# JihyongOh/DeMFI

Measured on AMD Instinct MI355X. Metric: interpolated frames/sec @720p x8 MFI (N_tst=3), higher is better.
Workload: dtype f16; 1 GPU; DeMFI-Net_rb N_tst=3, x8 MFI, 720x1280 (padded 736x1280), fp16, clip-parallel windows, random-init weights; uint8 frames host->HBM->host inside the timed region (PNG codec excluded), 8 distinct windows; graph=True, parallelism=clip1, n_ctx=7, n_trunk=3

## Files before the change

### demfi_amd/_lib.py

```python
import ctypes as C
import os

_HERE = os.path.dirname(os.path.abspath(__file__))
LIB_PATH = os.environ.get('DEMFI_HIP_LIB') or os.path.join(_HERE, 'csrc', 'libdemfi_hip.so')

F16, F32 = 0, 1
ABI_VERSION = 8
ACT_NONE, ACT_RELU, ACT_TANH, ACT_SIGMOID = 0, 1, 2, 3
MODE_STORE, MODE_MUL, MODE_GRU = 0, 1, 2
BT601, BT709 = 0, 1
SITING_420JPEG, SITING_420MPEG2 = 0, 1
YUV_LAYOUT = {'420': 0, '422': 1, '444': 2, 'mono': 3}
MAX_PIECES, MAX_CHUNKS, MAX_SEGS, MAX_OCTS = 48, 40, 8, 32


class View(C.Structure):
    _fields_ = [('ptr', C.c_void_p), ('sx', C.c_int64), ('sy', C.c_int64), ('sc', C.c_int64), ('sb', C.c_int64),
                ('is_f32', C.c_int32), ('_pad', C.c_int32)]


class Piece(C.Structure):
    _fields_ = [('v', View), ('nch', C.c_int32), ('lds_ch', C.c_int32), ('up_shift', C.c_int32), ('fat', C.c_int32)]


class Chunk(C.Structure):
    _fields_ = [('first_piece', C.c_int32), ('n_pieces', C.c_int32), ('nks', C.c_int32), ('_pad', C.c_int32),
                ('w_off', C.c_int64)]


class Seg(C.Structure):
    _fields_ = [('dst', View), ('res', View), ('aux', View), ('act', C.c_int32), ('mode', C.c_int32),
                ('scale', C.c_int32), ('dy', C.c_int32), ('dx', C.c_int32), ('_pad', C.c_int32)]


class Conv(C.Structure):
    _fields_ = [('dtype', C.c_int32), ('H', C.c_int32), ('W', C.c_int32), ('inH', C.c_int32), ('inW', C.c_int32),
                ('kh', C.c_int32), ('kw', C.c_int32), ('stride', C.c_int32), ('pad_y', C.c_int32),
                ('pad_x', C.c_int32), ('batch', C.c_int32), ('cout_pad', C.c_int32), ('nco', C.c_int32),
                ('rec_bytes', C.c_int32), ('n_chunks', C.c_int32), ('n_pieces', C.c_int32), ('n_segs', C.c_int32),
                ('cout_perm', C.c_int32), ('w_blk_stride', C.c_int64), ('wpack', C.c_void_p), ('bias', C.c_void_p), ('zero_page', C.c_void_p),
                ('chunks', Chunk * MAX_CHUNKS), ('pieces', Piece * MAX_PIECES), ('segs', Seg * MAX_SEGS),
                ('oct_seg', C.c_int32 * MAX_OCTS), ('oct_n', C.c_int32 * MAX_OCTS), ('oct_ch', C.c_int32 * MAX_OCTS),
                ('sub_seg', C.c_int32 * (MAX_OCTS // 4)),
                ('lw_magic', C.c_uint32), ('u8_iter', C.c_int32), ('u8_sink', C.c_void_p),
                ('pack', View), ('pack_oct_ch', C.c_int32 * 4)]


class U8Sink(C.Structure):
    _fields_ = [('frame', C.c_void_p * MAX_SEGS), ('h', C.c_int32), ('w', C.c_int32), ('iter', C.c_int32), ('_pad', C.c_int32)]


class ConvSrc(C.Structure):
    _fields_ = [('v', View), ('fat', C.c_int32), ('up_shift', C.c_int32), ('nch', C.c_int32), ('_pad', C.c_int32),
                ('cin', C.POINTER(C.c_int32))]


class ConvDst(C.Structure):
    _fields_ = [('dst', View), ('res', View), ('aux', View), ('act', C.c_int32), ('mode', C.c_int32), ('scale', C.c_int32),
                ('dy', C.c_int32), ('dx', C.c_int32), ('n', C.c_int32), ('couts', C.POINTER(C.c_int32))]


class HParams(C.Structure):
    _fields_ = [('nf', C.c_int32), ('scale_factor', C.c_int32), ('num_resb_facfb', C.c_int32), ('num_resb_dec', C.c_int32),
                ('shared_fgac', C.c_int32), ('fgac_rr', C.c_int32), ('fgac_sr', C.c_int32), ('flags', C.c_int32)]


class Batch(C.Structure):
    _fields_ = [('nb', C.c_int32), ('_pad', C.c_int32), ('a', C.c_int64), ('b', C.c_int64), ('o', C.c_int64), ('t', C.c_int64),
                ('p', C.c_int64 * 32)]


class Op(C.Structure):
    _fields_ = [('kind', C.c_int32), ('conv', C.c_int32), ('nch', C.c_int32), ('_pad', C.c_int32), ('macs', C.c_int64),
                ('a', View), ('b', View), ('o', View), ('p', C.c_void_p * 32), ('t', C.c_void_p), ('name', C.c_char * 64),
                ('bt', Batch)]


_SIGS = {
    'demfi_abi_version': (C.c_int, []),
    'demfi_last_error': (C.c_char_p, []),
    'demfi_device_info': (C.c_int, [C.c_char_p, C.c_int, C.POINTER(C.c_int), C.POINTER(C.c_int64)]),
    'demfi_pack_conv_weights': (C.c_int, [C.c_void_p, C.c_int, C.c_int, C.c_int, C.c_int, C.c_void_p, C.c_int,
                                          C.c_void_p, C.c_int, C.c_void_p, C.c_int, C.c_int, C.c_int, C.c_void_p,
                                          C.POINTER(C.c_int64)]),
    'demfi_conv_lds_bytes': (C.c_int64, [C.POINTER(Conv)]),
# ... 166 lines not shown
```

### demfi_amd/csrc/common.h

```cpp
#pragma once
#include <hip/hip_runtime.h>
#include <stdint.h>
#include <stdio.h>
#include "demfi_hip.h"

typedef _Float16 half_t;
typedef _Float16 h8_t __attribute__((ext_vector_type(8)));
typedef _Float16 h4_t __attribute__((ext_vector_type(4)));
typedef float f16x_t __attribute__((ext_vector_type(16)));
typedef float f4_t __attribute__((ext_vector_type(4)));

int demfi_set_error(int code, const char* fmt, ...);

struct demfi_conv;
bool demfi_persist_eligible(const demfi_conv* h);
bool demfi_ws2_eligible(const demfi_conv* h);
int demfi_ws2_launch(const demfi_conv* h, const demfi_conv* dev, void* stream);
#define DEMFI_HIP_CHECK(expr)                                                                   \
    do {                                                                                        \
        hipError_t e__ = (expr);                                                                \
        if (e__ != hipSuccess)                                                                  \
            return demfi_set_error(DEMFI_ERR_HIP, "%s failed: %s", #expr, hipGetErrorString(e__)); \
    } while (0)

#define DEMFI_GLOBAL __attribute__((address_space(1)))
template <typename T> __device__ __forceinline__ const DEMFI_GLOBAL T* gcp(const void* p) { return (const DEMFI_GLOBAL T*)p; }
template <typename T> __device__ __forceinline__ DEMFI_GLOBAL T* gp(void* p) { return (DEMFI_GLOBAL T*)p; }
typedef unsigned int u4_t __attribute__((ext_vector_type(4)));
__device__ __forceinline__ uint4 ld_global16(const void* p) { return __builtin_bit_cast(uint4, *gcp<u4_t>(p)); }
__device__ __forceinline__ void st_global16(void* p, const uint4& v) { *gp<u4_t>(p) = __builtin_bit_cast(u4_t, v); }
__device__ __forceinline__ void st_global16_nt(void* p, const uint4& v) { __builtin_nontemporal_store(__builtin_bit_cast(u4_t, v), gp<u4_t>(p)); }

__device__ __forceinline__ float view_load(const demfi_view& v, int64_t off)
{
    return v.is_f32 ? gcp<float>(v.ptr)[off] : (float)gcp<half_t>(v.ptr)[off];
}
__device__ __forceinline__ void view_store(const demfi_view& v, int64_t off, float x)
{
    if (v.is_f32) gp<float>(v.ptr)[off] = x;
    else gp<half_t>(v.ptr)[off] = (half_t)x;
}

__device__ __forceinline__ float sigmoidf_(float x) { return 1.0f / (1.0f + expf(-x)); }

__device__ __forceinline__ float fast_sigmoid(float x)
{
    return __builtin_amdgcn_rcpf(1.0f + __builtin_amdgcn_exp2f(-1.4426950408889634f * x));
}
__device__ __forceinline__ float fast_tanh(float x)
{
    return 1.0f - 2.0f * __builtin_amdgcn_rcpf(1.0f + __builtin_amdgcn_exp2f(2.8853900817779268f * x));
}

__device__ __forceinline__ float unnormalized_coord(float p, float den, float sizem1)
{
    float g = (2.0f * p) / den;
    g = g - 1.0f;
    float i = (g + 1.0f) / 2.0f;
    return i * sizem1;
}

struct SampleMap {
    int x0, y0;
    float w[4];
    int inb;
};

__device__ __forceinline__ SampleMap make_sample_map(float ix, float iy, int H, int W)
{
    SampleMap m;
// ... 30 lines not shown
```

### demfi_amd/csrc/conv.hip

```cpp
#include "conv_common.h"

namespace {

bool sep_eligible(const demfi_conv* h) { return demfi_sep_eligible(h); }
bool wstream_eligible(const demfi_conv* h, int ks = 7, int nch = 2) { return demfi_wstream_eligible(h, ks, nch); }

static bool persist_out_eligible(const demfi_conv* h, bool allow_tanh = false);

bool persist_eligible(const demfi_conv* h)
{
    if (h->dtype != DEMFI_F16 || h->stride != 1 || h->kh != 3 || h->kw != 3 || h->pad_y != 1 || h->pad_x != 1) return false;
    if (h->n_chunks != 1 || h->n_pieces != 1 || h->chunks[0].nks != 4 || h->rec_bytes != 128) return false;
    const demfi_piece& p = h->pieces[0];
    if (!p.fat || p.nch != 64 || p.up_shift != 0 || !p.v.ptr || p.v.is_f32) return false;
    return persist_out_eligible(h, h->nco == 2);
}

static bool thin_out_eligible(const demfi_conv* h)
{
    if (h->nco != 1 || h->cout_pad != 32 || !h->zero_page || h->inH != h->H || h->inW != h->W || h->sub_seg[0] >= 0) return false;
    bool any = false;
    for (int g = 0; g < 4; ++g) {
        if (h->oct_n[g] == 0) continue;
        any = true;
        const demfi_seg& sg = h->segs[h->oct_seg[g]];
        if (sg.mode != DEMFI_MODE_STORE || sg.scale != 1 || sg.dy != 0 || sg.dx != 0) return false;
        if (!sg.dst.ptr || !sg.dst.is_f32) return false;
        if (sg.res.ptr && !sg.res.is_f32) return false;
    }
    return any;
}

static bool narrow_eligible(const demfi_conv* h)
{
    if (h->dtype != DEMFI_F16 || h->stride != 1 || h->kh != h->kw || (h->kh != 3 && h->kh != 7) || h->pad_y != h->kh / 2 || h->pad_x != h->kw / 2)
        return false;
    if (h->n_chunks != 1) return false;
    const demfi_chunk& ch = h->chunks[0];
    if (ch.nks != 1 && ch.nks != 2 && ch.nks != 4) return false;
    if (h->kh == 7 && (ch.nks != 1 || h->nco != 1)) return false;
    int nreal = 0;
    for (int k = 0; k < ch.n_pieces; ++k) {
        const demfi_piece& p = h->pieces[ch.first_piece + k];
        if ((p.lds_ch * 2) % 16 || (p.nch * 2) % 16) return false;
        if (p.v.ptr == nullptr) continue;
        if (!p.fat || p.up_shift != 0 || p.v.is_f32 || p.v.sc != 1) return false;
        if (p.v.sy * 2 * 16 >= (int64_t)1 << 31 || p.v.sx * 2 * 64 >= (int64_t)1 << 31) return false;
        ++nreal;
    }
    if (nreal < 1 || nreal > 2) return false;
    return persist_out_eligible(h) || thin_out_eligible(h);
}

static bool persist_out_eligible(const demfi_conv* h, bool allow_tanh)
{
    if (h->nco > 2 || h->cout_pad != 32 * h->nco || !h->zero_page || h->inH != h->H || h->inW != h->W) return false;
    const int sg = h->sub_seg[0];
    if (sg < 0) return false;
    for (int sb = 0; sb < h->nco; ++sb)
        if (h->sub_seg[sb] != sg || h->oct_ch[sb * 4] != h->oct_ch[0] + 32 * sb) return false;
    const demfi_seg& seg = h->segs[sg];
    if (seg.mode != DEMFI_MODE_STORE || seg.scale != 1 || seg.dy != 0 || seg.dx != 0) return false;
    if (seg.act != DEMFI_ACT_NONE && seg.act != DEMFI_ACT_RELU && !(allow_tanh && seg.act == DEMFI_ACT_TANH)) return false;
    return true;
}

}


bool demfi_persist_eligible(const demfi_conv* h)
{
    return sep_eligible(h) || wstream_eligible(h) || wstream_eligible(h, 3, 1) || persist_eligible(h) || (narrow_eligible(h) && persist_out_eligible(h)) ||
           demfi_ws2_eligible(h);
}

extern "C" int64_t demfi_conv_lds_bytes(const demfi_conv* h)
{
    const int64_t LW = (int64_t)(TW - 1) * h->stride + h->kw;
    const int64_t LH = (int64_t)(TH - 1) * h->stride + h->kh;
    const int64_t tile = ((LW * LH * (h->rec_bytes + REC_PAD) + 1023) & ~1023ll)
                         + 2ll * (h->rec_bytes / 32) * h->nco * 1024;
    const int64_t stage = 4 * 64 * STAGE_LD * 4;
    return tile > stage ? tile : stage;
}

extern "C" int demfi_conv2d(const demfi_conv* h, const demfi_conv* dev, void* stream)
{
    if (!h || !dev) return demfi_set_error(DEMFI_ERR_ARG, "demfi_conv2d: null descriptor");
    if (h->dtype != DEMFI_F16 && h->dtype != DEMFI_F32) return demfi_set_error(DEMFI_ERR_ARG, "demfi_conv2d: dtype");
    if (h->stride != 1 && h->stride != 2) return demfi_set_error(DEMFI_ERR_ARG, "demfi_conv2d: stride %d", h->stride);
    if (h->cout_pad <= 0 || h->cout_pad > 256 || h->cout_pad % (32 * h->nco))
        return demfi_set_error(DEMFI_ERR_ARG, "demfi_conv2d: cout_pad=%d nco=%d", h->cout_pad, h->nco);
    if (h->rec_bytes != 32 && h->rec_bytes != 64 && h->rec_bytes != 128)
        return demfi_set_error(DEMFI_ERR_ARG, "demfi_conv2d: rec_bytes=%d", h->rec_bytes);
    if (h->n_chunks < 1 || h->n_chunks > DEMFI_MAX_CHUNKS || h->n_pieces > DEMFI_MAX_PIECES || h->n_segs > DEMFI_MAX_SEGS)
        return demfi_set_error(DEMFI_ERR_ARG, "demfi_conv2d: chunk/piece/seg count");
    const int64_t LW = (int64_t)(TW - 1) * h->stride + h->kw;
    const int64_t lds = demfi_conv_lds_bytes(h);
    if (lds > 160 * 1024) return demfi_set_error(DEMFI_ERR_ARG, "demfi_conv2d: LDS tile %lld B > 160 KiB", (long long)lds);
    if (LW * ((int64_t)(TH - 1) * h->stride + h->kh) >= 65536) return demfi_set_error(DEMFI_ERR_ARG, "demfi_conv2d: tile too large");
    if (h->lw_magic != (uint32_t)((0x100000000ull + LW - 1) / LW))
        return demfi_set_error(DEMFI_ERR_ARG, "demfi_conv2d: lw_magic mismatch");
    const int esz = h->dtype == DEMFI_F16 ? 2 : 4;
    for (int c = 0; c < h->n_chunks; ++c) {
        const demfi_chunk& ch = h->chunks[c];
        if (ch.nks < 1 || ch.nks * 32 > h->rec_bytes) return demfi_set_error(DEMFI_ERR_ARG, "demfi_conv2d: chunk %d nks", c);
        int used = 0;
        for (int pi = ch.first_piece; pi < ch.first_piece + ch.n_pieces; ++pi) {
            const demfi_piece& p = h->pieces[pi];
            if (p.lds_ch * esz != used) return demfi_set_error(DEMFI_ERR_ARG, "demfi_conv2d: piece %d not contiguous in chunk", pi);
            if (p.fat) {
                const int bytes = p.nch * esz, vpp = bytes / 16;
                if (bytes % 16 || (vpp & (vpp - 1)) || vpp > 8 || p.v.sc != 1 || (p.v.is_f32 != (h->dtype == DEMFI_F32)))
                    return demfi_set_error(DEMFI_ERR_ARG, "demfi_conv2d: fat piece %d malformed", pi);
            }
            used += p.nch * esz;
        }
        if (used != ch.nks * 32) return demfi_set_error(DEMFI_ERR_ARG, "demfi_conv2d: chunk %d covers %d B, expected %d", c, used, ch.nks * 32);
    }
    for (int sb = 0; sb < h->cout_pad / 32; ++sb) {
        const int sgi = h->sub_seg[sb];
        if (sgi < 0) continue;
        if (sgi >= h->n_segs) return demfi_set_error(DEMFI_ERR_ARG, "demfi_conv2d: sub_seg[%d]=%d", sb, sgi);
        const demfi_seg& sg = h->segs[sgi];
        const int f32 = h->dtype == DEMFI_F32;
        bool ok = sg.dst.ptr && sg.dst.sc == 1 && sg.dst.is_f32 == f32;
        if (sg.res.ptr) ok = ok && sg.res.sc == 1 && sg.res.is_f32 == f32;
        if (sg.mode == DEMFI_MODE_GRU) ok = ok && sg.aux.ptr && sg.aux.sc == 1 && sg.aux.is_f32 == f32;
        if (sg.mode != DEMFI_MODE_STORE) ok = ok && sg.res.ptr;
        for (int o = 0; o < 4; ++o)
            ok = ok && h->oct_seg[sb * 4 + o] == sgi && h->oct_n[sb * 4 + o] == 8 &&
                 h->oct_ch[sb * 4 + o] == h->oct_ch[sb * 4] + 8 * o;
        ok = ok && h->oct_ch[sb * 4] % 8 == 0;
        if (!ok) return demfi_set_error(DEMFI_ERR_ARG, "demfi_conv2d: subtile %d is not eligible for the staged epilogue", sb);
    }
    hipStream_t st = (hipStream_t)stream;
    if (h->pack.ptr != nullptr) {
        bool ok = h->dtype == DEMFI_F16 && narrow_eligible(h) && thin_out_eligible(h) && !persist_out_eligible(h) && h->pack.sc == 1 && !h->pack.is_f32;
        for (int g = 0; g < 4; ++g) ok = ok && (h->pack_oct_ch[g] < 0 || (h->pack_oct_ch[g] % 4 == 0 && h->oct_n[g] > 0));
        if (!ok) return demfi_set_error(DEMFI_ERR_ARG, "demfi_conv2d: packed copy (demfi_conv.pack) on a layer that is not a thin-output fp16 narrow layer, or malformed");
    }
    if ((h->cout_perm != 0) != demfi_persist_eligible(h))
        return demfi_set_error(DEMFI_ERR_ARG, h->cout_perm ? "demfi_conv2d: descriptor packed for a persistent kernel (cout_perm) but not eligible for one (zero_page missing?)"
                                                           : "demfi_conv2d: persistent-kernel layer without cout_perm (build the descriptor with demfi_conv_build)");
    if (sep_eligible(h)) return demfi_sep_launch(h, dev, st);
    if (wstream_eligible(h)) return demfi_wstream_launch(h, dev, st);
    if (!persist_eligible(h) && !narrow_eligible(h) && demfi_ws2_eligible(h)) return demfi_ws2_launch(h, dev, st);
    if (wstream_eligible(h, 3, 1)) return demfi_wstream3_launch(h, dev, st);
    if (persist_eligible(h)) return demfi_c64_launch(h, dev, st);
    if (narrow_eligible(h)) {
        bool handled = false;
        const int rc = demfi_narrow_launch(h, dev, st, !persist_out_eligible(h), &handled);
        if (handled) return rc;
    }
    return demfi_conv_general_launch(h, dev, st, (size_t)lds);
}

#ifdef DEMFI_TRACE
extern "C" int demfi_trace_dump(unsigned long long* out, int64_t n)
{
    const int64_t have = (int64_t)TR_WGS * TR_WAVES * TR_TILES * TR_STAMPS;
    if (!out || n < have) return demfi_set_error(DEMFI_ERR_ARG, "demfi_trace_dump: need room for %lld entries", (long long)have);
    DEMFI_HIP_CHECK(hipDeviceSynchronize());
    for (int64_t i = 0; i < have; ++i) out[i] = 0;
    int st = demfi_c64_trace_collect(out);
    if (st >= 0) st = demfi_narrow_trace_collect(out);
    if (st >= 0) st = demfi_sep_trace_collect(out);
    if (st >= 0) st = demfi_wstream_trace_collect(out);
    return st < 0 ? st : (int)have;
}
#endif
```

### demfi_amd/csrc/ctx.cpp

```cpp
#include "common.h"
#include <algorithm>
#include <map>
#include <set>
#include <string>
#include <stdlib.h>
#include <string.h>
#include <vector>

namespace {

constexpr int64_t LDS_BUDGET = 78 * 1024;

struct BuiltConv {
    demfi_conv d;
    std::vector<uint8_t> wpack;
    std::vector<float> bias;
    int64_t wbytes = 0;
    int64_t macs = 0;
};

int build_conv(int dtype, int H, int W, int stride, int batch, const float* w, const float* bias, int cout, int cin, int kh,
               int kw, const demfi_conv_src* srcs, int n_srcs, const demfi_conv_dst* dsts, int n_dsts, BuiltConv& out,
               bool size_only, const char* name, int pad_y = -1, int pad_x = -1, int grid_div = 1)
{
    if (dtype != DEMFI_F16 && dtype != DEMFI_F32) return demfi_set_error(DEMFI_ERR_ARG, "%s: dtype", name);
    if (!srcs || !dsts || n_srcs <= 0 || n_dsts <= 0 || n_dsts > DEMFI_MAX_SEGS || (stride != 1 && stride != 2))
        return demfi_set_error(DEMFI_ERR_ARG, "%s: sources / destinations / stride", name);
    const int esz = dtype == DEMFI_F32 ? 4 : 2;
    const int64_t LH = 7 * stride + kh, LW = 31 * stride + kw;
    int n_oct = 0;
    for (int i = 0; i < n_dsts; ++i) n_oct += (dsts[i].n + 7) / 8;
    const int sub = (n_oct + 3) / 4;
    int nco = sub <= 5 ? sub : 4;
    int rec = 128;
    int src_nch = 0;
    for (int i = 0; i < n_srcs; ++i) src_nch += srcs[i].nch;
    const bool ws2_s2 = stride == 2 && kh == 4 && kw == 4, ws2_s1 = stride == 1 && kh == 3 && kw == 3 && src_nch > 64;
    bool ws2_shape = esz == 2 && (ws2_s2 || ws2_s1) && pad_y < 0 && pad_x < 0 && n_dsts == 1 && dsts[0].n % 64 == 0 &&
                     dsts[0].mode == DEMFI_MODE_STORE && (dsts[0].act == DEMFI_ACT_NONE || dsts[0].act == DEMFI_ACT_RELU) && dsts[0].scale <= 1 &&
                     dsts[0].dst.sc == 1 && !dsts[0].dst.is_f32 && (!dsts[0].res.ptr || (dsts[0].res.sc == 1 && !dsts[0].res.is_f32));
    for (int i = 0; ws2_shape && i < n_srcs; ++i)
        ws2_shape = srcs[i].fat && !srcs[i].v.is_f32 &&
                    (srcs[i].nch % 32 == 0 || (srcs[i].nch == 16 && !srcs[i].up_shift && (i == n_srcs - 1 || (i == n_srcs - 2 && srcs[n_srcs - 1].nch == 8))) ||
                     (srcs[i].nch == 8 && !srcs[i].up_shift && i == n_srcs - 1 && i > 0 && srcs[i - 1].nch == 16)) &&
                    (srcs[i].up_shift == 0 || (srcs[i].up_shift == 1 && ws2_s1 && H % 2 == 0 && W % 2 == 0));
    if (ws2_shape) nco = 2;
    bool sep = esz == 2 && stride == 1 && ((kh == 1 && kw == 5) || (kh == 5 && kw == 1)) && n_srcs == 2 && (cout == 64 || cout == 128);
    for (int i = 0; sep && i < n_srcs; ++i) sep = srcs[i].fat && srcs[i].nch == 64 && !srcs[i].up_shift;
    while (!sep && rec > 32 && LH * LW * (rec + 16) + 2 * (rec / 32) * nco * 1024 > LDS_BUDGET) rec /= 2;
    {
        const int64_t n_wg = (int64_t)((W + 31) / 32) * ((H + 7) / 8) * (batch / grid_div) * ((sub + nco - 1) / nco);
        const bool persist_shape = n_srcs == 1 && srcs[0].fat && srcs[0].nch == 64 && kh == 3 && kw == 3 && stride == 1;
        if (!sep && !persist_shape && rec == 128 && nco <= 2 && n_wg <= 5 * 256) rec = 64;
        bool rdb_shape = !sep && esz == 2 && kh == 3 && kw == 3 && stride == 1 && sub == 1 && n_dsts == 1 && dsts[0].n == 32 && cin >= 96 && pad_y < 0 && pad_x < 0;
        for (int i = 0; rdb_shape && i < n_srcs; ++i) rdb_shape = srcs[i].fat && !srcs[i].up_shift && srcs[i].nch % 32 == 0;
        if (rdb_shape || ws2_shape) rec = 64;
    }

    {
        std::vector<int> seen(cin, 0);
        for (int i = 0; i < n_srcs; ++i)
            for (int j = 0; j < srcs[i].nch; ++j) {
                const int c = srcs[i].cin[j];
                if (c >= cin) return demfi_set_error(DEMFI_ERR_ARG, "%s: input map names channel %d >= cin %d", name, c, cin);
                if (c >= 0) seen[c]++;
            }
        for (int c = 0; c < cin; ++c)
            if (seen[c] != 1) return demfi_set_error(DEMFI_ERR_ARG, "%s: input channel %d fed %d times", name, c, seen[c]);
    }
    struct P { demfi_view v; int nch, lds_ch, up, fat; };
    struct Ck { int first, n, nks; };
    std::vector<P> pieces;
    std::vector<Ck> chunks;
    std::vector<int32_t> cin_map;
    int first = 0, fill = 0;
    const demfi_view null_view = {nullptr, 0, 0, 0, 0, 0, 0};
    auto close_chunk = [&]() {
        if (fill == 0) return;
        const int unit = ws2_shape ? 64 : 32;
        const int padb = (unit - fill % unit) % unit;
        if (padb) {
            pieces.push_back({null_view, padb / esz, fill / esz, 0, 0});
            cin_map.insert(cin_map.end(), padb / esz, -1);
            fill += padb;
        }
        chunks.push_back({first, (int)pieces.size() - first, fill / 32});
        first = (int)pieces.size();
        fill = 0;
    };
    std::vector<int> order;
    for (int i = 0; i < n_srcs; ++i) if (srcs[i].fat) order.push_back(i);
    for (int i = 0; i < n_srcs; ++i) if (!srcs[i].fat) order.push_back(i);
    for (int si : order) {
        const demfi_conv_src& s = srcs[si];
        const int selt = s.v.is_f32 ? 4 : 2;
        int done = 0;
        while (done < s.nch) {
            if (fill >= rec) close_chunk();
            const int room = (rec - fill) / esz;
// ... 975 lines not shown
        OpList& th = tb > 1 ? c->tb_head_ops[k] : c->head_ops[k][q];
        const int H = c->H, W = c->W, N = c->N;
        const int H2 = H / 2, W2 = W / 2, H4 = H / 4, W4 = W / 4, H8 = H / 8, W8 = W / 8;
        const int R = DEMFI_ACT_RELU, T = DEMFI_ACT_TANH;
        const int64_t hw4 = (int64_t)H * W * 4;
        const Tensor& ffo = TB["ffo"];
        const Tensor& aF = TB["aF"];
        const Tensor& x = TB["x"];
        const void* tp = ptr(B["t"]);
        auto delta_v = [&](int step, int ch) { return tview(B["delta"], 5 * step + ch); };
        auto delta_p = [&](int step, int ch) { return plane(B["delta"], 5 * step + ch); };
        {
            demfi_op o = blank();
            o.p[0] = ptr(ffo); o.p[1] = ptr(ffo) + 2 * hw4; o.p[2] = ptr(B["cfr_acc"]); o.p[3] = ptr(B["ft"]); o.t = tp;
            o.p[4] = ptr(ffo) + 4 * hw4; o.p[5] = ptr(B["misc16"]);
            simple(th, DEMFI_OP_CFR, "cfr", o);
        }
        warp(th, "warp_fat", 64, fview(TB["F01"], 0, 0), fview(TB["F01"], 0, 1), fview(B["Ft"], 0, 0), ptr(B["ft"]), ptr(B["ft"]) + 2 * hw4,
             ptr(ffo) + 4 * hw4, nullptr, tp);
        std::string p = "Refine_Module.";
        {
            std::vector<int32_t> m = range(192, 201);
            m.insert(m.end(), 7, -1);
            if (c->dtype == DEMFI_F16) {
                std::vector<int32_t> sel = range(128, 201), m2 = range(64, 73);
                m2.insert(m2.end(), 7, -1);
                SubW wb = sub_weight(p + "enc1", sel, false);
                conv(th, p + "enc1#t", {fsrc(B["Ft"], 0), fsrc_map(B["misc16"], m2)},
                     {D(fview(B["u1"]), range(0, 64), R, DEMFI_MODE_STORE, fview(TB["u1a"]))}, H2, W2, 2, 1, &wb.w, &wb.b, &wb.shape);
            } else
            conv(th, p + "enc1", {fsrc(aF, 0, 0, -1, 0), fsrc(aF, 64, 0, -1, 1), fsrc(B["Ft"], 128), fsrc_map(B["misc16"], m)},
                 {D(fview(B["u1"]), range(0, 64), R)}, H2, W2, 2);
        }
        conv(th, p + "enc2", {fsrc(B["u1"], 0)}, {D(fview(B["u2"]), range(0, 128), R)}, H4, W4, 2);
        conv(th, p + "enc3", {fsrc(B["u2"], 0)}, {D(fview(B["u3"]), range(0, 256), R)}, H8, W8, 2);
        conv(th, p + "dec0", {fsrc(B["u3"], 0)}, {D(fview(B["d0"]), range(0, 256), R)}, H8, W8);
        conv(th, p + "dec1", {fsrc(B["d0"], 0, 0, -1, -1, 1), fsrc(B["u2"], 256)}, {D(fview(B["d1"]), range(0, 128), R)}, H4, W4);
        conv(th, p + "dec2", {fsrc(B["d1"], 0, 0, -1, -1, 1), fsrc(B["u1"], 128)}, {D(fview(B["d2"]), range(0, 64), R)}, H2, W2);
        if (c->dtype == DEMFI_F16) {
            auto it = c->table.find(p + "dec3");
            const Layer l3 = it->second;
            auto iw = c->weights.find(p + "dec3.weight"), ib = c->weights.find(p + "dec3.bias");
            if (!dry && (iw == c->weights.end() || ib == c->weights.end())) {
                status = demfi_set_error(DEMFI_ERR_ARG, "demfi_ctx_bind: weight '%s' was not loaded", (p + "dec3").c_str());
                return;
            }
            auto phase_view = [&](demfi_view v, int dy, int dx) {
                const int64_t elt = v.is_f32 ? 4 : 2;
                v.ptr = (char*)v.ptr + ((int64_t)dy * v.sy + (int64_t)dx * v.sx) * elt;
                v.sx *= 2; v.sy *= 2;
                return v;
            };
            const Layer l9 = {l3.cout, l3.cin, 3, 3};
            for (int dy = 0; dy < 2 && status >= 0; ++dy) {
                std::vector<float> wf2, bf2;
                for (int dx = 0; dx < 2 && status >= 0; ++dx) {
                    std::vector<float> w9e, b2;
                    if (!dry) {
                        w9e.assign((size_t)l3.cout * l3.cin * 9, 0.0f);
                        for (int co = 0; co < l3.cout; ++co)
                            for (int ci = 0; ci < l3.cin; ++ci) {
                                const float* w9 = &iw->second.data[((size_t)co * l3.cin + ci) * 9];
                                float* we = &w9e[((size_t)co * l3.cin + ci) * 9];
                                for (int ky = 0; ky < 3; ++ky)
                                    for (int kx = 0; kx < 3; ++kx) {
                                        const int a = dy == 0 ? (ky >= 1) : (ky >= 2), b = dx == 0 ? (kx >= 1) : (kx >= 2);
                                        we[(a + dy) * 3 + (b + dx)] += w9[ky * 3 + kx];
                                    }
                            }
                        b2 = ib->second.data;
                    }
                    const std::string nm = p + "dec3#p" + std::to_string(dy) + std::to_string(dx);
                    auto slice = [&](int c0, int c1, std::vector<float>& w, std::vector<float>& b) {
                        if (dry) return;
                        w.assign(w9e.begin() + (size_t)c0 * l3.cin * 9, w9e.begin() + (size_t)c1 * l3.cin * 9);
                        b.assign(b2.begin() + c0, b2.begin() + c1);
                    };
                    std::vector<float> wa, ba, wb, bb, wf, bf;
                    slice(5, 69, wa, ba); slice(69, 133, wb, bb); slice(0, 5, wf, bf);
                    const Layer l64 = {64, l3.cin, 3, 3};
                    conv(th, nm + "a", {fsrc(B["d2"], 0)},
                         {D(phase_view(fview(B["rF"], 0, 0), dy, dx), range(0, 64), T, DEMFI_MODE_STORE, phase_view(fview(aF, 0, 0), dy, dx))},
                         H2, W2, 1, 1, &wa, &ba, &l64);
                    conv(th, nm + "b", {fsrc(B["d2"], 0)},
                         {D(phase_view(fview(B["rF"], 0, 1), dy, dx), range(0, 64), T, DEMFI_MODE_STORE, phase_view(fview(aF, 0, 1), dy, dx))},
                         H2, W2, 1, 1, &wb, &bb, &l64);
                    wf2.insert(wf2.end(), wf.begin(), wf.end());
                    bf2.insert(bf2.end(), bf.begin(), bf.end());
                }
                if (status >= 0) {
                    const Layer l10 = {10, l3.cin, 3, 3};
                    pack_next(phase_view(fview(B["delta16"]), dy, 0), 0, 4, 16, 20);
                    conv(th, p + "dec3#p" + std::to_string(dy) + "xf", {fsrc(B["d2"], 0)},
                         {D(phase_view(delta_v(0, 0), dy, 0), range(0, 4), DEMFI_ACT_NONE, DEMFI_MODE_STORE, phase_view(tview(B["ft"]), dy, 0)),
                          D(phase_view(delta_v(0, 4), dy, 0), {4}, DEMFI_ACT_NONE, DEMFI_MODE_STORE, phase_view(tview(ffo, 4), dy, 0)),
                          D(phase_view(delta_v(0, 0), dy, 1), range(5, 9), DEMFI_ACT_NONE, DEMFI_MODE_STORE, phase_view(tview(B["ft"]), dy, 1)),
                          D(phase_view(delta_v(0, 4), dy, 1), {9}, DEMFI_ACT_NONE, DEMFI_MODE_STORE, phase_view(tview(ffo, 4), dy, 1))},
                         H2, W2, 1, 1, &wf2, &bf2, &l10);
                }
            }
        } else
        conv(th, p + "dec3", {fsrc(B["d2"], 0, 0, -1, -1, 1)},
             {D(fview(B["rF"], 0, 0), range(5, 69), T, DEMFI_MODE_STORE, fview(aF, 0, 0)),
              D(fview(B["rF"], 0, 1), range(69, 133), T, DEMFI_MODE_STORE, fview(aF, 0, 1)),
              D(delta_v(0, 0), range(0, 4), DEMFI_ACT_NONE, DEMFI_MODE_STORE, tview(B["ft"])),
              D(delta_v(0, 4), {4}, DEMFI_ACT_NONE, DEMFI_MODE_STORE, tview(ffo, 4))}, H, W);
        warp(th, "warp_fat", 64, fview(B["rF"], 0, 0), fview(B["rF"], 0, 1), fview(B["rF"], 0, 2), delta_p(0, 0), delta_p(0, 2),
             delta_p(0, 4), plane(B["occ"], 0), tp);
        conv(th, "Dec_first", {fsrc(B["rF"], 0)}, {D(fview(B["dec_a"]), range(0, 64), R)}, H, W, 1, 3);
        const Tensor* cur = resblocks(th, "Decoder_res", c->hp.num_resb_dec, B["dec_a"], B["dec_t"], B["dec_b"], H, W, 3);
        conv(th, "Dec_last1", {fsrc(*cur, 0)}, {D(fview(B["dec_t"]), range(0, 64), R)}, H, W, 1, 3);
        conv(th, "Dec_last2", {fsrc(B["dec_t"], 0)}, {D(tview(B["sharp1"], 0, 3ll * H * W), range(0, 3))}, H, W, 1, 3);
        conv(th, "Ch_Reducer", {fsrc(B["rF"], 0, 0, -1, 0), fsrc(B["rF"], 64, 0, -1, 1), fsrc(B["rF"], 128, 0, -1, 2)},
             {D(fview(B["frec0"]), range(0, 64), T)}, H, W);
        p = "Booster_Module.";
        std::vector<const float*> xpl;
        for (int f = 0; f < 4; ++f)
            for (int col = 0; col < 3; ++col) xpl.push_back(plane(x, col * 4 + f));
        std::vector<int32_t> agg3s_cin = range(0, 6);
        if (c->dtype == DEMFI_F16) {
            std::vector<const float*> pl;
            for (int i = 0; i < 9; ++i) pl.push_back(plane(B["sharp1"], i));
            for (int i = 0; i < 5; ++i) pl.push_back(delta_p(0, i));
            pl.push_back(plane(B["occ"], 0));
            pack(th, pl, B["ref16"]);
            std::vector<int32_t> sel = range(0, 9), m = range(0, 14);
            for (int i = 25; i < 30; ++i) sel.push_back(i);
            m.insert(m.end(), 2, -1);
            SubW w1 = sub_weight(p + "Mixer.conv_ref1", sel, true);
            conv(th, p + "Mixer.conv_ref1#t", {fsrc_map(B["ref16"], m)}, {D(fview(B["re1"]), range(0, 32), R, DEMFI_MODE_STORE, fview(TB["re1w"]))},
                 H, W, 1, 1, &w1.w, &w1.b, &w1.shape);
        } else {
            {
                std::vector<const float*> pl;
                for (int i = 0; i < 9; ++i) pl.push_back(plane(B["sharp1"], i));
                pl.insert(pl.end(), xpl.begin(), xpl.end());
                for (int i : {2, 3, 0, 1}) pl.push_back(plane(ffo, i));
                for (int i = 0; i < 5; ++i) pl.push_back(delta_p(0, i));
                pack(th, pl, B["ref32"]);
                std::vector<int32_t> m = range(0, 30);
                m.insert(m.end(), 2, -1);
// ... 713 lines not shown
```

### demfi_amd/csrc/wsconv.hip

```cpp
#include "common.h"
#include <type_traits>
#include <stdlib.h>
#include <string.h>

namespace {

template <int I, int N, typename F>
__device__ __forceinline__ void ws_for(F&& f)
{
    if constexpr (I < N) {
        f(std::integral_constant<int, I>{});
        ws_for<I + 1, N>(f);
    }
}
__device__ __forceinline__ void ws_mma(f16x_t& acc, const uint4& a, const uint4& b)
{
    acc = __builtin_amdgcn_mfma_f32_32x32x16_f16(__builtin_bit_cast(h8_t, a), __builtin_bit_cast(h8_t, b), acc, 0, 0, 0);
}

template <bool S2, int NCH = 2> struct Ws2Cfg {
    static constexpr int KSE = S2 ? 2 : 3;
    static constexpr int RPW = 8;
    static constexpr int TH = RPW * (4 / NCH), TWP = 32;
    static constexpr int LH = TH + KSE - 1, LL = TWP + KSE - 1;
// ... 444 lines not shown
        k.res = sg.res.ptr ? (const char*)sg.res.ptr + (int64_t)ch0 * 2 : nullptr;
        k.r_sb = sg.res.sb * 2; k.r_sx = (int)(sg.res.sx * 2); k.r_sy = (int)(sg.res.sy * 2);
        k.relu = sg.act == DEMFI_ACT_RELU;
    }
    for (int c = 0; c < h->n_chunks; ++c) {
        const demfi_chunk& ch = h->chunks[c];
        const demfi_piece& p = h->pieces[ch.first_piece];
        WsChunk& k = a.ch[c];
        k.src = (const char*)p.v.ptr; k.sb = p.v.sb * 2; k.sx = (int)(p.v.sx * 2); k.sy = (int)(p.v.sy * 2);
        k.flags = (p.nch == 16 ? 1 : 0) | (p.up_shift ? 2 : 0);
        k.w_off = (int)(ch.w_off * 16);
        if (ch.n_pieces == 3) {
            const demfi_piece& q = h->pieces[ch.first_piece + 1];
            k.src2 = (const char*)q.v.ptr; k.sb2 = q.v.sb * 2; k.sx2 = (int)(q.v.sx * 2); k.sy2 = (int)(q.v.sy * 2);
        }
    }
    const int grid = total >= 256 ? 256 : (int)total;
    static const bool tracing = getenv("DEMFI_WS2_TRACE") && atoi(getenv("DEMFI_WS2_TRACE")) != 0;
    static unsigned long long* trbuf = nullptr;
    if (tracing) {
        if (!trbuf) { DEMFI_HIP_CHECK(hipMalloc(&trbuf, 8 * 512 * 8)); }
        DEMFI_HIP_CHECK(hipMemset(trbuf, 0, 8 * 512 * 8));
        a.trace = trbuf;
    }
    constexpr int lds_s2 = Ws2Cfg<true, 2>::LDS_BYTES, lds_3 = Ws2Cfg<false, 2>::LDS_BYTES, lds_31 = Ws2Cfg<false, 1>::LDS_BYTES;
    if (h->stride == 2) {
        DEMFI_LDS_ATTR((conv_ws2_kernel<true, 2>));
        hipLaunchKernelGGL((conv_ws2_kernel<true, 2>), dim3(grid), dim3(WS_NTHREADS), lds_s2, (hipStream_t)stream, a);
    } else if (nco == 2) {
        DEMFI_LDS_ATTR((conv_ws2_kernel<false, 2>));
        hipLaunchKernelGGL((conv_ws2_kernel<false, 2>), dim3(grid), dim3(WS_NTHREADS), lds_3, (hipStream_t)stream, a);
    } else {
        DEMFI_LDS_ATTR((conv_ws2_kernel<false, 1>));
        hipLaunchKernelGGL((conv_ws2_kernel<false, 1>), dim3(grid), dim3(WS_NTHREADS), lds_31, (hipStream_t)stream, a);
    }
    DEMFI_HIP_CHECK(hipGetLastError());
    if (tracing) {
        static unsigned long long host[8 * 512];
        DEMFI_HIP_CHECK(hipStreamSynchronize((hipStream_t)stream));
        DEMFI_HIP_CHECK(hipMemcpy(host, trbuf, sizeof(host), hipMemcpyDeviceToHost));
        for (int w : {0, 4}) {
            fprintf(stderr, "[ws2 trace] stride %d chunks %d blocks %d wave %d:", h->stride, h->n_chunks, h->cout_pad / (32 * nco), w);
            unsigned long long prev = 0;
            for (int i = 0; i < 512 && host[w * 512 + i]; ++i) {
                const unsigned long long t = host[w * 512 + i] & 0xffffffffffffffull;
                fprintf(stderr, " %d:%lld", (int)(host[w * 512 + i] >> 56), prev ? (long long)(t - prev) : 0ll);
                prev = t;
            }
            fprintf(stderr, "\n");
        }
    }
    return DEMFI_OK;
}
```

### include/demfi_hip.h

```cpp
#ifndef DEMFI_HIP_H
#define DEMFI_HIP_H

#include <stdint.h>

#ifdef __cplusplus
extern "C" {
#endif

#define DEMFI_ABI_VERSION 8

enum demfi_dtype { DEMFI_F16 = 0, DEMFI_F32 = 1 };

enum demfi_status {
    DEMFI_OK = 0,
    DEMFI_ERR_ARG = -1,
    DEMFI_ERR_HIP = -2,
    DEMFI_ERR_NODEV = -3
};

enum demfi_yuv_matrix { DEMFI_BT601 = 0, DEMFI_BT709 = 1 };
enum demfi_chroma_siting { DEMFI_420JPEG = 0, DEMFI_420MPEG2 = 1 };
enum demfi_yuv_layout { DEMFI_YUV_420 = 0, DEMFI_YUV_422 = 1, DEMFI_YUV_444 = 2, DEMFI_YUV_MONO = 3 };

enum demfi_act { DEMFI_ACT_NONE = 0, DEMFI_ACT_RELU = 1, DEMFI_ACT_TANH = 2, DEMFI_ACT_SIGMOID = 3 };

enum demfi_mode { DEMFI_MODE_STORE = 0, DEMFI_MODE_MUL = 1, DEMFI_MODE_GRU = 2 };

typedef struct demfi_view {
    void*   ptr;
    int64_t sx;
    int64_t sy;
    int64_t sc;
    int64_t sb;
    int32_t is_f32;
    int32_t _pad;
} demfi_view;

typedef struct demfi_piece {
    demfi_view v;
    int32_t nch;
    int32_t lds_ch;
    int32_t up_shift;
    int32_t fat;
} demfi_piece;

#define DEMFI_MAX_PIECES 48
#define DEMFI_MAX_CHUNKS 40
#define DEMFI_MAX_SEGS    8
#define DEMFI_MAX_OCTS   32

typedef struct demfi_chunk {
    int32_t first_piece;
    int32_t n_pieces;
    int32_t nks;
    int32_t _pad;
    int64_t w_off;
} demfi_chunk;

typedef struct demfi_seg {
    demfi_view dst;
    demfi_view res;
    demfi_view aux;
    int32_t act;
    int32_t mode;
    int32_t scale;
    int32_t dy, dx;
    int32_t _pad;
} demfi_seg;

typedef struct demfi_conv {
    int32_t dtype;
    int32_t H, W;
    int32_t inH, inW;
    int32_t kh, kw;
    int32_t stride;
    int32_t pad_y, pad_x;
    int32_t batch;
    int32_t cout_pad;
    int32_t nco;
    int32_t rec_bytes;
    int32_t n_chunks;
    int32_t n_pieces;
    int32_t n_segs;
    int32_t cout_perm;
    int64_t w_blk_stride;
    const void*  wpack;
    const float* bias;
    const void*  zero_page;
    demfi_chunk chunks[DEMFI_MAX_CHUNKS];
    demfi_piece pieces[DEMFI_MAX_PIECES];
    demfi_seg   segs[DEMFI_MAX_SEGS];
    int32_t oct_seg[DEMFI_MAX_OCTS];
    int32_t oct_n[DEMFI_MAX_OCTS];
    int32_t oct_ch[DEMFI_MAX_OCTS];
    int32_t sub_seg[DEMFI_MAX_OCTS / 4];
    uint32_t lw_magic;
    int32_t  u8_iter;
    const struct demfi_u8_sink* u8_sink;
    demfi_view pack;
    int32_t pack_oct_ch[4];
} demfi_conv;

#define DEMFI_U8_SINK_STRIDE 256
typedef struct demfi_u8_sink {
    uint8_t* frame[DEMFI_MAX_SEGS];
    int32_t  h, w;
    int32_t  iter;
    int32_t  _pad;
} demfi_u8_sink;

int         demfi_abi_version(void);
const char* demfi_last_error(void);
int         demfi_device_info(char* name, int len, int* n_cu, int64_t* hbm_bytes);

int demfi_pack_conv_weights(const float* w_oihw, int cout, int cin, int kh, int kw,
                            const int32_t* cin_map, int n_k, const int32_t* chunk_nks, int n_chunks,
                            const int32_t* cout_map, int cout_pad, int nco, int dtype,
                            void* out, int64_t* out_bytes);

int64_t demfi_conv_lds_bytes(const demfi_conv* host_desc);
// ... 224 lines not shown
```

Before: 104.1 frames/s.

## Fuse dec3 phase convs into one 256-channel kernel sharing the input tile

For each output row parity, the two per-column-phase 64-channel dec3 convolutions (a and b) for both column phases are merged into a single 256-output conv. A new MFMA kernel stages the input tile into LDS once, then loops over four 64-channel blocks, each using its own 2x2 tap footprint, fused residual add and tanh. The goal is to cut repeated input loads and kernel launches across the four separate convs. It adds a new segment field and a dedicated, narrowly eligible kernel path, and the old path stays available through an environment variable.

```diff
diff --git a/demfi_amd/_lib.py b/demfi_amd/_lib.py
--- a/demfi_amd/_lib.py
+++ b/demfi_amd/_lib.py
@@ -30,7 +30,7 @@
 
 class Seg(C.Structure):
     _fields_ = [('dst', View), ('res', View), ('aux', View), ('act', C.c_int32), ('mode', C.c_int32),
-                ('scale', C.c_int32), ('dy', C.c_int32), ('dx', C.c_int32), ('_pad', C.c_int32)]
+                ('scale', C.c_int32), ('dy', C.c_int32), ('dx', C.c_int32), ('taps2x2', C.c_int32)]
 
 
 class Conv(C.Structure):
diff --git a/demfi_amd/csrc/common.h b/demfi_amd/csrc/common.h
--- a/demfi_amd/csrc/common.h
+++ b/demfi_amd/csrc/common.h
@@ -16,6 +16,8 @@
 bool demfi_persist_eligible(const demfi_conv* h);
 bool demfi_ws2_eligible(const demfi_conv* h);
 int demfi_ws2_launch(const demfi_conv* h, const demfi_conv* dev, void* stream);
+bool demfi_dec3_eligible(const demfi_conv* h);
+int demfi_dec3_launch(const demfi_conv* h, const demfi_conv* dev, void* stream);
 #define DEMFI_HIP_CHECK(expr)                                                                   \
     do {                                                                                        \
         hipError_t e__ = (expr);                                                                \
diff --git a/demfi_amd/csrc/conv.hip b/demfi_amd/csrc/conv.hip
--- a/demfi_amd/csrc/conv.hip
+++ b/demfi_amd/csrc/conv.hip
@@ -71,7 +71,7 @@
 bool demfi_persist_eligible(const demfi_conv* h)
 {
     return sep_eligible(h) || wstream_eligible(h) || wstream_eligible(h, 3, 1) || persist_eligible(h) || (narrow_eligible(h) && persist_out_eligible(h)) ||
-           demfi_ws2_eligible(h);
+           demfi_ws2_eligible(h) || demfi_dec3_eligible(h);
 }
 
 extern "C" int64_t demfi_conv_lds_bytes(const demfi_conv* h)
@@ -146,6 +146,7 @@
     if (sep_eligible(h)) return demfi_sep_launch(h, dev, st);
     if (wstream_eligible(h)) return demfi_wstream_launch(h, dev, st);
     if (!persist_eligible(h) && !narrow_eligible(h) && demfi_ws2_eligible(h)) return demfi_ws2_launch(h, dev, st);
+    if (demfi_dec3_eligible(h)) return demfi_dec3_launch(h, dev, st);
     if (wstream_eligible(h, 3, 1)) return demfi_wstream3_launch(h, dev, st);
     if (persist_eligible(h)) return demfi_c64_launch(h, dev, st);
     if (narrow_eligible(h)) {
diff --git a/demfi_amd/csrc/ctx.cpp b/demfi_amd/csrc/ctx.cpp
--- a/demfi_amd/csrc/ctx.cpp
+++ b/demfi_amd/csrc/ctx.cpp
@@ -45,6 +45,11 @@
                      (srcs[i].nch == 8 && !srcs[i].up_shift && i == n_srcs - 1 && i > 0 && srcs[i - 1].nch == 16)) &&
                     (srcs[i].up_shift == 0 || (srcs[i].up_shift == 1 && ws2_s1 && H % 2 == 0 && W % 2 == 0));
     if (ws2_shape) nco = 2;
+    bool dec3_shape = esz == 2 && stride == 1 && kh == 3 && kw == 3 && pad_y < 0 && pad_x < 0 && n_srcs == 1 && srcs[0].fat && srcs[0].nch == 64 &&
+                      !srcs[0].up_shift && n_dsts == 4;
+    for (int i = 0; dec3_shape && i < n_dsts; ++i)
+        dec3_shape = dsts[i].n == 64 && dsts[i].mode == DEMFI_MODE_STORE && dsts[i].act == DEMFI_ACT_TANH && dsts[i].scale <= 1 && dsts[i].res.ptr;
+    if (dec3_shape) nco = 2;
     bool sep = esz == 2 && stride == 1 && ((kh == 1 && kw == 5) || (kh == 5 && kw == 1)) && n_srcs == 2 && (cout == 64 || cout == 128);
     for (int i = 0; sep && i < n_srcs; ++i) sep = srcs[i].fat && srcs[i].nch == 64 && !srcs[i].up_shift;
     while (!sep && rec > 32 && LH * LW * (rec + 16) + 2 * (rec / 32) * nco * 1024 > LDS_BUDGET) rec /= 2;
@@ -1126,8 +1131,9 @@
                 return v;
             };
             const Layer l9 = {l3.cout, l3.cin, 3, 3};
+            const bool fused3 = !(getenv("DEMFI_DEC3_FUSED") && atoi(getenv("DEMFI_DEC3_FUSED")) == 0);
             for (int dy = 0; dy < 2 && status >= 0; ++dy) {
-                std::vector<float> wf2, bf2;
+                std::vector<float> wf2, bf2, w256, b256;
                 for (int dx = 0; dx < 2 && status >= 0; ++dx) {
                     std::vector<float> w9e, b2;
                     if (!dry) {
@@ -1153,14 +1159,29 @@
                     std::vector<float> wa, ba, wb, bb, wf, bf;
                     slice(5, 69, wa, ba); slice(69, 133, wb, bb); slice(0, 5, wf, bf);
                     const Layer l64 = {64, l3.cin, 3, 3};
+                    w256.insert(w256.end(), wa.begin(), wa.end()); w256.insert(w256.end(), wb.begin(), wb.end());
+                    b256.insert(b256.end(), ba.begin(), ba.end()); b256.insert(b256.end(), bb.begin(), bb.end());
+                    if (!fused3) {
                     conv(th, nm + "a", {fsrc(B["d2"], 0)},
                          {D(phase_view(fview(B["rF"], 0, 0), dy, dx), range(0, 64), T, DEMFI_MODE_STORE, phase_view(fview(aF, 0, 0), dy, dx))},
                          H2, W2, 1, 1, &wa, &ba, &l64);
                     conv(th, nm + "b", {fsrc(B["d2"], 0)},
                          {D(phase_view(fview(B["rF"], 0, 1), dy, dx), range(0, 64), T, DEMFI_MODE_STORE, phase_view(fview(aF, 0, 1), dy, dx))},
                          H2, W2, 1, 1, &wb, &bb, &l64);
+                    }
                     wf2.insert(wf2.end(), wf.begin(), wf.end());
                     bf2.insert(bf2.end(), bf.begin(), bf.end());
+                }
+                if (status >= 0 && fused3) {
+                    const Layer l256 = {256, l3.cin, 3, 3};
+                    std::vector<Dst> ds;
+                    for (int dx = 0; dx < 2; ++dx)
+                        for (int hf = 0; hf < 2; ++hf)
+                            ds.push_back(D(phase_view(fview(B["rF"], 0, hf), dy, dx), range(64 * (2 * dx + hf), 64 * (2 * dx + hf) + 64), T, DEMFI_MODE_STORE,
+                                           phase_view(fview(aF, 0, hf), dy, dx)));
+                    conv(th, p + "dec3#p" + std::to_string(dy), {fsrc(B["d2"], 0)}, ds, H2, W2, 1, 1, &w256, &b256, &l256);
+                    if (status >= 0)
+                        for (int s = 0; s < 4; ++s) c->descs.back().segs[s].taps2x2 = 1 + 2 * dy + (s >> 1);
                 }
                 if (status >= 0) {
                     const Layer l10 = {10, l3.cin, 3, 3};
diff --git a/demfi_amd/csrc/wsconv.hip b/demfi_amd/csrc/wsconv.hip
--- a/demfi_amd/csrc/wsconv.hip
+++ b/demfi_amd/csrc/wsconv.hip
@@ -520,3 +520,259 @@
     }
     return DEMFI_OK;
 }
+
+namespace {
+
+struct D3Cfg {
+    static constexpr int TH = 16, TWP = 32, RPW = 8;
+    static constexpr int LH = TH + 1, LL = TWP + 2;
+    static constexpr int NREC = LH * LL;
+    static constexpr int NI = (NREC + 7) / 8;
+    static constexpr int NIW = (NI + 3) / 4;
+    static constexpr int LDS_BYTES = NIW * 4 * 1024;
+    static constexpr int NTHREADS = 256;
+    static_assert(2 * LDS_BYTES <= 160 * 1024, "two workgroups per CU");
+};
+struct D3Block {
+    char* dst; const char* res;
+    int64_t d_sb, r_sb;
+    int d_sx, d_sy, r_sx, r_sy;
+    int dx, _pad;
+};
+struct D3Args {
+    const char* src; const char* wpack; const float* bias; const char* zeros;
+    int64_t s_sb, w_blk_stride;
+    int s_sx, s_sy, H, W, batch, dy;
+    D3Block blk[4];
+};
+
+__global__ __launch_bounds__(D3Cfg::NTHREADS, 2) void conv_dec3_kernel(const D3Args a)
+{
+    using C = D3Cfg;
+    constexpr int RPW = C::RPW;
+    extern __shared__ __attribute__((aligned(16))) char smem[];
+    const int tid = threadIdx.x;
+    const int lane = tid & 63;
+    const int wave = __builtin_amdgcn_readfirstlane(tid >> 6);
+    const int H = a.H, W = a.W, dy = a.dy;
+    const int tiles_x = (W + C::TWP - 1) / C::TWP, tiles_y = (H + C::TH - 1) / C::TH, tiles_img = tiles_x * tiles_y;
+    const int total = tiles_img * a.batch;
+    int it0, it1;
+    {
+        const int G = gridDim.x;
+        if ((G & 7) == 0 && total >= G) {
+            const int xcd = blockIdx.x & 7, idx = blockIdx.x >> 3, nw = G >> 3;
+            const int q = total >> 3, r = total & 7;
+            const int lo = xcd * q + min(xcd, r), n = q + (xcd < r ? 1 : 0);
+            it0 = lo + (int)(((int64_t)n * idx) / nw);
+            it1 = lo + (int)(((int64_t)n * (idx + 1)) / nw);
+        } else {
+            it0 = (int)(((int64_t)total * blockIdx.x) / G);
+            it1 = (int)(((int64_t)total * (blockIdx.x + 1)) / G);
+        }
+    }
+    if (it0 >= it1) return;
+    const char* const zeros = a.zeros;
+    auto tile_pos = [&](int t, int& img, int& oy0, int& ox0) {
+        img = t / tiles_img;
+        const int rem = t - img * tiles_img;
+        const int ty = rem / tiles_x;
+        oy0 = ty * C::TH;
+        ox0 = (rem - ty * tiles_x) * C::TWP;
+    };
+    auto issue_tile = [&](int t) {
+        int img, oy0, ox0;
+        tile_pos(t, img, oy0, ox0);
+        const int iy0 = oy0 - 1 + dy, ix0 = ox0 - 1;
+        const char* const base = a.src + img * a.s_sb + (int64_t)iy0 * a.s_sy + (int64_t)ix0 * a.s_sx;
+#pragma unroll
+        for (int j = 0; j < C::NIW; ++j) {
+            const int i = wave + 4 * j;
+            const int rec = i * 8 + (lane >> 3);
+            const int l = rec / C::LL, c = rec - l * C::LL;
+            const int v = (lane & 7) ^ ((c >> 1) & 7);
+            const int iy = iy0 + l, ix = ix0 + c;
+            const bool ok = rec < C::NREC && (unsigned)iy < (unsigned)H && (unsigned)ix < (unsigned)W;
+            const char* g = ok ? base + (unsigned)(l * a.s_sy + c * a.s_sx + v * 16) : zeros;
+            __builtin_amdgcn_global_load_lds((const DEMFI_GLOBAL void*)g, (__attribute__((address_space(3))) void*)(smem + i * 1024), 16, 0, 0);
+        }
+    };
+
+    const int hi = lane >> 5, lx = lane & 31;
+    const int cs = wave & 1, rh = wave >> 1;
+    const unsigned lane16 = lane * 16;
+    struct Step { int img, oy0, ox0, blk; };
+    auto step_at = [&](int t, int blk) { Step s; tile_pos(t, s.img, s.oy0, s.ox0); s.blk = blk; return s; };
+    auto a_base = [&](const Step& s) {
+        const char* wb = a.wpack + s.blk * a.w_blk_stride + (((dy * 3 + a.blk[s.blk].dx) * 4) * 2 + cs) * 1024;
+        asm volatile("" : "+s"(wb));
+        return wb;
+    };
+    auto a_load = [&](const char* wb, int kx2, int ks, int ky2) {
+        return __builtin_bit_cast(uint4, *gcp<u4_t>(wb + (unsigned)((((ky2 * 3 + kx2) * 4 + ks) * 2) * 1024 + lane16)));
+    };
+    auto res_fetch = [&](const Step& s, int p0, u4_t (&rr)[4][2]) {
+        const D3Block& bk = a.blk[s.blk];
+        const int ox = min(s.ox0 + lx, W - 1);
+        const char* const rb = bk.res + s.img * bk.r_sb + cs * 64;
+        const unsigned loff = (unsigned)(ox * bk.r_sx + hi * 16);
+#pragma unroll
+        for (int p = 0; p < 4; ++p) {
+            const int oy = min(s.oy0 + rh * RPW + p0 + p, H - 1);
+            const char* const row = rb + (int64_t)oy * bk.r_sy;
+#pragma unroll
+            for (int m2 = 0; m2 < 2; ++m2) rr[p][m2] = *gcp<u4_t>(row + (loff + m2 * 32));
+        }
+    };
+
+    f16x_t acc[RPW];
+    auto finish_rows = [&](const Step& s, int p0, const u4_t (&rr)[4][2]) {
+        const D3Block& bk = a.blk[s.blk];
+        const int ox = s.ox0 + lx;
+        const int oyb = s.oy0 + rh * RPW + p0;
+        char* const ob = bk.dst + s.img * bk.d_sb + (int64_t)oyb * bk.d_sy + cs * 64;
+        const unsigned loff = (unsigned)(ox * bk.d_sx + hi * 16);
+#pragma unroll
+        for (int p = 0; p < 4; ++p) {
+#pragma unroll
+            for (int m2 = 0; m2 < 2; ++m2) {
+                float v[8];
+#pragma unroll
+                for (int j = 0; j < 4; ++j) {
+                    v[j] = acc[p0 + p][(2 * m2) * 4 + j];
+                    v[4 + j] = acc[p0 + p][(2 * m2 + 1) * 4 + j];
+                }
+                const u4_t r = rr[p][m2];
+#pragma unroll
+                for (int q = 0; q < 4; ++q) {
+                    v[2 * q] = ws_mix_lo(r[q], v[2 * q]);
+                    v[2 * q + 1] = ws_mix_hi(r[q], v[2 * q + 1]);
+                }
+                h8_t o;
+#pragma unroll
+                for (int j = 0; j < 8; ++j) o[j] = (half_t)fast_tanh(v[j]);
+                if (oyb + p < H && ox < W) *gp<h8_t>(ob + p * bk.d_sy + (loff + m2 * 32)) = o;
+            }
+        }
+    };
+
+    issue_tile(it0);
+    Step cur = step_at(it0, 0);
+    u4_t rr_lo[4][2];
+    uint4 A0[2];
+    {
+        const char* wb = a_base(cur);
+        A0[0] = a_load(wb, 0, 0, 0);
+        A0[1] = a_load(wb, 0, 0, 1);
+        res_fetch(cur, 0, rr_lo);
+    }
+    for (int t = it0; t < it1; ++t) {
+        asm volatile("s_waitcnt vmcnt(0)" ::: "memory");
+        asm volatile("s_barrier" ::: "memory");
+#pragma unroll 1
+        for (int blk = 0; blk < 4; ++blk) {
+            const bool more = blk < 3 || t + 1 < it1;
+            const Step nxt = blk < 3 ? Step{cur.img, cur.oy0, cur.ox0, blk + 1} : (more ? step_at(t + 1, 0) : cur);
+            const int dx = a.blk[blk].dx;
+            const char* const wb = a_base(cur);
+            {
+                f4_t bq[4];
+#pragma unroll
+                for (int qd = 0; qd < 4; ++qd) bq[qd] = *gcp<f4_t>(a.bias + blk * 64 + cs * 32 + qd * 8 + hi * 4);
+#pragma unroll
+                for (int p = 0; p < RPW; ++p) {
+#pragma unroll
+                    for (int qd = 0; qd < 4; ++qd) {
+#pragma unroll
+                        for (int j = 0; j < 4; ++j) acc[p][qd * 4 + j] = bq[qd][j];
+                    }
+                }
+            }
+            uint4 A[2] = {A0[0], A0[1]};
+            ws_for<0, 8>([&](auto G_) {
+                constexpr int g = decltype(G_)::value, kx2 = g >> 2, ks = g & 3;
+                const int col = lx + kx2 + dx;
+                const char* const tb = smem + (rh * RPW * C::LL + col) * 128 + ((((ks * 2 + hi) ^ ((col >> 1) & 7))) << 4);
+                uint4 B[RPW + 1];
+                ws_for<0, RPW + 1>([&](auto L_) { B[decltype(L_)::value] = *(const uint4*)(tb + decltype(L_)::value * (C::LL * 128)); });
+                uint4 An[2];
+                if constexpr (g < 7) {
+                    An[0] = a_load(wb, (g + 1) >> 2, (g + 1) & 3, 0);
+                    An[1] = a_load(wb, (g + 1) >> 2, (g + 1) & 3, 1);
+                }
+                ws_for<0, RPW>([&](auto P) { ws_mma(acc[decltype(P)::value], A[0], B[decltype(P)::value]); });
+                ws_for<0, RPW>([&](auto P) { ws_mma(acc[decltype(P)::value], A[1], B[decltype(P)::value + 1]); });
+                if constexpr (g < 7) { A[0] = An[0]; A[1] = An[1]; }
+            });
+            u4_t rr_hi[4][2];
+            res_fetch(cur, 4, rr_hi);
+            if (more) {
+                const char* wn = a_base(nxt);
+                A0[0] = a_load(wn, 0, 0, 0);
+                A0[1] = a_load(wn, 0, 0, 1);
+            }
+            finish_rows(cur, 0, rr_lo);
+            if (more) res_fetch(nxt, 0, rr_lo);
+            finish_rows(cur, 4, rr_hi);
+            if (blk == 3 && t + 1 < it1) {
+                asm volatile("s_barrier" ::: "memory");
+                issue_tile(t + 1);
+            }
+            cur = nxt;
+        }
+    }
+}
+
+}
+
+bool demfi_dec3_eligible(const demfi_conv* h)
+{
+    if (h->dtype != DEMFI_F16 || !h->zero_page || h->stride != 1 || h->kh != 3 || h->kw != 3 || h->pad_y != 1 || h->pad_x != 1) return false;
+    if (h->inH != h->H || h->inW != h->W || h->n_chunks != 1 || h->n_pieces != 1 || h->chunks[0].nks != 4 || h->rec_bytes != 128) return false;
+    if (h->nco != 2 || h->cout_pad != 256 || h->n_segs != 4 || h->u8_sink || h->pack.ptr) return false;
+    const demfi_piece& p = h->pieces[0];
+    if (!p.fat || p.nch != 64 || p.up_shift != 0 || !p.v.ptr || p.v.is_f32 || p.v.sc != 1) return false;
+    if (p.v.sy * 2 * 40 + p.v.sx * 2 * 40 >= (int64_t)1 << 31) return false;
+    if (h->w_blk_stride * 16 * 4 >= (int64_t)1 << 31) return false;
+    for (int b = 0; b < 4; ++b) {
+        if (h->sub_seg[2 * b] != b || h->sub_seg[2 * b + 1] != b) return false;
+        for (int o = 0; o < 8; ++o)
+            if (h->oct_seg[8 * b + o] != b || h->oct_n[8 * b + o] != 8 || h->oct_ch[8 * b + o] != h->oct_ch[8 * b] + 8 * o) return false;
+        const demfi_seg& sg = h->segs[b];
+        if (sg.mode != DEMFI_MODE_STORE || sg.act != DEMFI_ACT_TANH || sg.scale != 1 || sg.dy || sg.dx || sg.aux.ptr) return false;
+        if (!sg.dst.ptr || sg.dst.is_f32 || sg.dst.sc != 1 || !sg.res.ptr || sg.res.is_f32 || sg.res.sc != 1) return false;
+        if (sg.dst.sy * 2 * 20 + sg.dst.sx * 2 * 40 >= (int64_t)1 << 31 || sg.res.sy * 2 * 20 + sg.res.sx * 2 * 40 >= (int64_t)1 << 31) return false;
+    }
+    return true;
+}
+
+int demfi_dec3_launch(const demfi_conv* h, const demfi_conv* , void* stream)
+{
+    using C = D3Cfg;
+    const int64_t total = (int64_t)((h->W + C::TWP - 1) / C::TWP) * ((h->H + C::TH - 1) / C::TH) * h->batch;
+    if (total <= 0 || total >= (int64_t)1 << 30) return demfi_set_error(DEMFI_ERR_ARG, "demfi_conv2d (dec3 kernel): empty or oversized launch");
+    if (!h->wpack || !h->bias) return demfi_set_error(DEMFI_ERR_ARG, "demfi_conv2d (dec3 kernel): weights / bias not bound");
+    D3Args a;
+    memset(&a, 0, sizeof(a));
+    const demfi_piece& p = h->pieces[0];
+    a.src = (const char*)p.v.ptr; a.s_sb = p.v.sb * 2; a.s_sx = (int)(p.v.sx * 2); a.s_sy = (int)(p.v.sy * 2);
+    a.wpack = (const char*)h->wpack; a.bias = h->bias; a.zeros = (const char*)h->zero_page;
+    a.w_blk_stride = h->w_blk_stride * 16;
+    a.H = h->H; a.W = h->W; a.batch = h->batch;
+    for (int b = 0; b < 4; ++b) {
+        const demfi_seg& sg = h->segs[b];
+        if (sg.taps2x2 < 1 || sg.taps2x2 > 4 || (b > 0 && ((sg.taps2x2 - 1) >> 1) != a.dy))
+            return demfi_set_error(DEMFI_ERR_ARG, "demfi_conv2d (dec3 kernel): segment %d does not name its 2x2 tap footprint (demfi_seg.taps2x2), or the row parities differ", b);
+        a.dy = (sg.taps2x2 - 1) >> 1;
+        const int ch0 = h->oct_ch[8 * b];
+        D3Block& k = a.blk[b];
+        k.dx = (sg.taps2x2 - 1) & 1;
+        k.dst = (char*)sg.dst.ptr + (int64_t)ch0 * 2; k.d_sb = sg.dst.sb * 2; k.d_sx = (int)(sg.dst.sx * 2); k.d_sy = (int)(sg.dst.sy * 2);
+        k.res = (const char*)sg.res.ptr + (int64_t)ch0 * 2; k.r_sb = sg.res.sb * 2; k.r_sx = (int)(sg.res.sx * 2); k.r_sy = (int)(sg.res.sy * 2);
+    }
+    const int grid = total >= 512 ? 512 : (int)total;
+    DEMFI_LDS_ATTR(conv_dec3_kernel);
+    hipLaunchKernelGGL(conv_dec3_kernel, dim3(grid), dim3(C::NTHREADS), C::LDS_BYTES, (hipStream_t)stream, a);
+    DEMFI_HIP_CHECK(hipGetLastError());
+    return DEMFI_OK;
+}
diff --git a/include/demfi_hip.h b/include/demfi_hip.h
--- a/include/demfi_hip.h
+++ b/include/demfi_hip.h
@@ -65,7 +65,7 @@
     int32_t mode;
     int32_t scale;
     int32_t dy, dx;
-    int32_t _pad;
+    int32_t taps2x2;
 } demfi_seg;
 
 typedef struct demfi_conv {
```

Result: no change. 103.2 frames/s (-0.9%).
